# tingliu/glia

Measured on AMD Instinct MI355X. Metric: region_merges_per_sec, higher is better.
Workload: dtype u32 labels / f32 image / f64 statistics and features

## Files before the change

### glia_amd/csrc/api.cpp

```cpp
#include <algorithm>
#include <atomic>
#include <cmath>
#include <cstdlib>
#include <cstring>
#include <limits>
#include <mutex>
#include <unordered_map>

#include "rmap_order.hpp"
#include "api_types.hpp"

namespace glia {

static thread_local std::string g_err;
void set_error(const std::string& msg) { g_err = msg; }

static const char* const kOptionKeys[] = {"GLIA_HMT_PB_WINDOW", "GLIA_HMT_PB_BATCH", "GLIA_HMT_WINCAP", "GLIA_HMT_REBASE", "GLIA_HMT_HORIZON",
                                          "GLIA_HMT_FORCE_TREE", "GLIA_HMT_HELPERS", "GLIA_HMT_TRACE", "GLIA_HMT_LIBM", "GLIA_HMT_BC_NOCOMMON",
                                          "GLIA_HMT_BC_GENERIC", "GLIA_HMT_DEBUG", "GLIA_HMT_MAXITERS", "GLIA_HMT_MINCAP", "GLIA_HMT_MEDIAN_BATCH", "GLIA_HMT_BCFEAT", "GLIA_HMT_CC",
                                          "GLIA_HMT_TRAIN_TREES"};
static std::mutex g_opt_mu;
static std::unordered_map<std::string, std::string> g_opt;
static bool g_opt_init = false;
static void opt_init_locked() {
  if (g_opt_init) return;
  for (const char* k : kOptionKeys) if (const char* e = getenv(k)) g_opt[k] = e;
  g_opt_init = true;
}
static bool opt_known(const char* key) { for (const char* k : kOptionKeys) if (!strcmp(k, key)) return true; return false; }
bool option(const char* key, std::string* value) {
  std::lock_guard<std::mutex> lock(g_opt_mu);
  opt_init_locked();
  auto it = g_opt.find(key);
  if (it == g_opt.end()) return false;
  if (value) *value = it->second;
  return true;
}
int set_option(const char* key, const char* value) {
  if (!key || !opt_known(key)) { set_error(std::string("set_option: unknown option ") + (key ? key : "(null)")); return GLIA_HMT_ERR_ARG; }
  std::lock_guard<std::mutex> lock(g_opt_mu);
  opt_init_locked();
  if (value) g_opt[key] = value; else g_opt.erase(key);
  return GLIA_HMT_OK;
}

float ceil_f32(double d) {
  if (std::isinf(d) || std::isnan(d)) return (float)d;
  float f = (float)d;
  if ((double)f < d) f = std::nextafterf(f, std::numeric_limits<float>::infinity());
  return f;
}
static float floor_f32(double d) {
  if (std::isinf(d) || std::isnan(d)) return (float)d;
// ... 333 lines not shown
```

### glia_amd/csrc/greedy.hip

```cpp
#include <atomic>
#include <cstring>
#include <vector>
#include <limits>
#include <rocprim/device/device_scan.hpp>
#include <rocprim/device/device_radix_sort.hpp>
#include <rocprim/device/device_segmented_radix_sort.hpp>

#include "greedy_batch.hpp"

namespace glia {

__global__ void pq_build_level_kernel(PqTree t, int l) {
  const int lane = threadIdx.x & 63;
  uint32_t j = (blockIdx.x * blockDim.x + threadIdx.x) >> 6;
  if (j < t.lv[l].size) (void)pq_recompute_node(t, l, j, lane, true);
}

int pq_setup(DeviceBuffers& buf, PqTree& t, hipStream_t stream) {
  t.nlevels = 0;
  uint32_t n = t.nleaves;
  while (true) {
    n = (n + kFan - 1) / kFan;
    if (t.nlevels >= kMaxLevels) { set_error("greedy: edge table too large"); return GLIA_HMT_ERR_ARG; }
    PqLevel& L = t.lv[t.nlevels++];
// ... 14 lines not shown
  for (int l = 0; l < t.nlevels; ++l) {
    unsigned long long threads = (unsigned long long)t.lv[l].size * 64ull;
    hipLaunchKernelGGL(pq_build_level_kernel, dim3((unsigned)((threads + 255) / 256)), dim3(256), 0, stream, t, l);
  }
  GLIA_HIP_TRY(hipGetLastError());
  return GLIA_HMT_OK;
}

namespace {

__global__ void win_range_kernel(const double* sal, uint32_t E0, unsigned long long* mm) {
  unsigned long long lo = ~0ull, hi = 0ull;
  for (uint32_t i = blockIdx.x * blockDim.x + threadIdx.x; i < E0; i += gridDim.x * blockDim.x) {
    const unsigned long long b = f64_ord(sal[i]);
    lo = b < lo ? b : lo; hi = b > hi ? b : hi;
  }
  atomicMin(&mm[0], lo); atomicMax(&mm[1], hi);
}
__global__ void win_params_kernel(const unsigned long long* mm, uint32_t B, double* range) {
  const double smin = f64_unord(mm[0]), smax = f64_unord(mm[1]);
  range[0] = smin;
  range[1] = smax > smin ? (double)B / (smax - smin) : 0.0;
}
__global__ void win_collect_kernel(const EdgeRec* er, uint32_t n_edges, const uint8_t* rdead, unsigned long long* kseq, uint32_t* vals, uint32_t* counter) {
  const uint32_t e = blockIdx.x * blockDim.x + threadIdx.x;
  if (e >= n_edges) return;
  const unsigned long long q = er[e].seq;
  if (q == 0) return;
  const uint2 uv = *reinterpret_cast<const uint2*>(&er[e].u);
  if (rdead[uv.x] | rdead[uv.y]) return;
  const uint32_t i = atomicAdd(counter, 1u);
  kseq[i] = q; vals[i] = e;
}
__global__ void win_collect_lists_kernel(WinState st, uint32_t n_regions, unsigned long long* kseq, uint32_t* vals, uint32_t cap, uint32_t* counter) {
  const uint32_t r = (blockIdx.x * blockDim.x + threadIdx.x) >> 6, lane = threadIdx.x & 63u;
  if (r >= n_regions || st.rdead[r]) return;
  const uint32_t off = st.adj_off[r], len = st.adj_len[r];
  const double smin = st.wrange[0], scale = st.wrange[1];
  uint32_t rebuilt = 0;
  for (uint32_t base = 0; base < len; base += 64u) {
    const uint32_t i = base + lane;
    unsigned long long q = 0;
    uint32_t e = kNone;
    if (i < len) {
      const FatEntry fe = st.fpool[off + i];
      if (fe.eid != kNone && fe.rs < r && !st.rdead[fe.rs]) {
        e = fe.eid;
        if ((unsigned long long)e >= st.ne_base && win_cell(-fe.mean, smin, scale, st.wB) < st.wch) {
          const EdgeRec rec = rebuild_edge_record(fe, i, r, off, len, st.ecat[e], st.R0);
          st.er[e] = rec;
          q = rec.seq; ++rebuilt;
        } else q = st.er[e].seq;
      }
    }
    const unsigned long long m = __ballot(q != 0);
    if (m == 0) continue;
    const int first = (int)__builtin_ctzll(m);
    uint32_t b0 = 0;
    if ((int)lane == first) b0 = atomicAdd(&counter[0], (uint32_t)__popcll(m));
    b0 = (uint32_t)__shfl((int)b0, first);
    const uint32_t o = b0 + (uint32_t)__popcll(m & ((1ull << lane) - 1ull));
    if (q != 0 && o < cap) { kseq[o] = q; vals[o] = e; }
  }
  if (rebuilt) atomicAdd(&counter[1], rebuilt);
}
__global__ void win_salkey_kernel(const EdgeRec* er, const uint32_t* vals, uint32_t n, unsigned long long* ksal) {
  const uint32_t i = blockIdx.x * blockDim.x + threadIdx.x;
  if (i < n) ksal[i] = f64_ord(er[vals[i]].sal);
}
__global__ void win_baseline_fill_kernel(WinState st, uint32_t n, uint32_t* isort_w, unsigned long long* isort_seq) {
  const uint32_t i = blockIdx.x * blockDim.x + threadIdx.x;
  if (i >= n) return;
  const EdgeRec r = st.er[isort_w[i]];
  isort_seq[i] = r.seq;
  atomicAdd(&st.wcnt[win_cell(r.sal, st.wrange[0], st.wrange[1], st.wB)], 1u);
}
__global__ void win_segments_kernel(WinState st, const uint32_t* isort, uint32_t n, uint32_t* ige) {
  const uint32_t c = blockIdx.x * blockDim.x + threadIdx.x;
  if (c > st.wB) return;
  uint32_t lo = 0, hi = n;
  while (lo < hi) {
    const uint32_t mid = (lo + hi) >> 1;
    if (win_cell(st.er[isort[mid]].sal, st.wrange[0], st.wrange[1], st.wB) >= c) lo = mid + 1; else hi = mid;
  }
  ige[c] = c == 0 ? n : lo;
}
__global__ void adj_fill_fat(GreedyState g, WinState st, uint32_t E0, uint32_t* cursor) {
  const uint32_t e = blockIdx.x * blockDim.x + threadIdx.x;
  if (e >= E0) return;
  const uint32_t u = g.e_u[e], v = g.e_v[e];
  const uint32_t pu = atomicAdd(&cursor[u], 1u), pv = atomicAdd(&cursor[v], 1u);
  const uint32_t ou = g.adj_off[u], ov = g.adj_off[v], lu = g.adj_len[u], lv = g.adj_len[v];
  FatEntry a; a.eid = e; a.rs = v; a.n = (uint32_t)g.e_n[e]; a.pos = pv; a.off = ov; a.len = lv; a.mean = g.e_mean[e];
  FatEntry b = a; b.rs = u; b.pos = pu; b.off = ou; b.len = lu;
  st.fpool[ou + pu] = a; g.e_posu[e] = pu;
  st.fpool[ov + pv] = b; g.e_posv[e] = pv;
  EdgeRec r; r.u = u; r.v = v; r.posu = pu; r.posv = pv; r.mean = g.e_mean[e]; r.n = g.e_n[e]; r.next = kNone;
  r.hu = make_uint2(ou, lu); r.hv = make_uint2(ov, lv); r.sal = g.pq.leaf_sal[e]; r.seq = g.pq.leaf_seq[e];
  st.er[e] = r;
}
__global__ void fat_to_thin(const FatEntry* f, uint2* out, unsigned long long n) {
  const unsigned long long i = (unsigned long long)blockIdx.x * blockDim.x + threadIdx.x;
  if (i < n) { const FatEntry fe = f[i]; out[i] = make_uint2(fe.eid, fe.eid == kNone ? 0u : fe.rs); }
}
__global__ void edge_unpack(GreedyState g, const EdgeRec* er, const uint8_t* rdead, uint32_t n) {
  const uint32_t e = blockIdx.x * blockDim.x + threadIdx.x;
  if (e >= n) return;
  const EdgeRec r = er[e];
  g.e_u[e] = r.u; g.e_v[e] = r.v; g.e_posu[e] = r.posu; g.e_posv[e] = r.posv; g.e_mean[e] = r.mean; g.e_n[e] = r.n;
  g.pq.leaf_sal[e] = r.sal; g.pq.leaf_seq[e] = (rdead[r.u] | rdead[r.v]) ? 0ull : r.seq;
}

__global__ void edge_unpack_live(GreedyState g, const EdgeRec* er, const uint32_t* vals, uint32_t n) {
  const uint32_t i = blockIdx.x * blockDim.x + threadIdx.x;
  if (i >= n) return;
  const uint32_t e = vals[i];
  const EdgeRec r = er[e];
  g.e_u[e] = r.u; g.e_v[e] = r.v; g.e_posu[e] = r.posu; g.e_posv[e] = r.posv; g.e_mean[e] = r.mean; g.e_n[e] = r.n;
// ... 79 lines not shown
__global__ void median_from_runs(const unsigned long long* pv_off, const float* pv, unsigned long long nV, const uint32_t* pa, const uint32_t* pb, long long P,
                                 const uint32_t* flag, const uint32_t* eidx, const unsigned long long* e_off, float* out) {
  const unsigned long long v = (unsigned long long)blockIdx.x * blockDim.x + threadIdx.x;
  if (v >= nV) return;
  long long lo = 0, hi = P;
  while (lo < hi) { const long long mid = (lo + hi) >> 1; if (pv_off[mid + 1] <= v) lo = mid + 1; else hi = mid; }
  const long long i = lo;
  const uint32_t a = pa[i], b = pb[i];
  const long long owner = a < b ? i : find_pair(pa, pb, P, b, a);
  if (owner < 0 || !flag[owner]) return;
  const unsigned long long first = owner == i ? 0ull : pv_off[owner + 1] - pv_off[owner];
  out[e_off[eidx[owner]] + first + (v - pv_off[i])] = pv[v];
}

__global__ void median_init(GreedyState st, uint32_t E0) {
  const uint32_t e = blockIdx.x * blockDim.x + threadIdx.x;
  if (e >= E0) return;
  const uint32_t n = (uint32_t)st.e_n[e];
  const double med = (double)st.vals[st.e_off[e] + n / 2u];
  st.e_mean[e] = med;
  st.pq.leaf_sal[e] = st.size_weight ? -med * (double)min(st.rsz[st.e_u[e]], st.rsz[st.e_v[e]]) : -med;
  atomicAdd(&st.rbv[st.e_u[e]], (unsigned long long)n);
  atomicAdd(&st.rbv[st.e_v[e]], (unsigned long long)n);
}

__global__ void fill_leaves_dead(PqTree t, uint32_t from) {
  uint32_t i = from + blockIdx.x * blockDim.x + threadIdx.x;
  if (i < t.nleaves) { t.leaf_seq[i] = 0; t.leaf_sal[i] = -__builtin_inf(); }
}

}

struct WinBaseline {
  unsigned long long *kseq = nullptr, *kseq2 = nullptr, *ksal = nullptr, *ksal2 = nullptr, *iseq = nullptr;
  uint32_t *vals = nullptr, *vals2 = nullptr, *isort = nullptr, *ige = nullptr, *counter = nullptr;
  void* tmp = nullptr; size_t tmp_bytes = 0;
  uint32_t E0 = 0;
  double h_range[2] = {0.0, 0.0};
  long long prev_top_cell = -1;
  unsigned long long prev_ne = 0;
  double horizon_factor = 0.0;
  bool from_lists = false;
  unsigned long long rebuilt_last = 0;

  int init(DeviceBuffers& buf, WinState& ws, const double* leaf_sal, uint32_t n_initial, uint32_t B, uint32_t R, hipStream_t stream) {
    int rc;
    E0 = n_initial;
    unsigned long long* mm; double* range;
    if ((rc = buf.get(&ws.rdead, 2 * (size_t)R, true, stream))) return rc;
    if ((rc = buf.get(&ws.whead, B, false, stream))) return rc;
    if ((rc = buf.get(&ws.wcnt, B, true, stream))) return rc;
    if ((rc = buf.get(&isort, E0, false, stream))) return rc;
    if ((rc = buf.get(&iseq, E0, false, stream))) return rc;
    if ((rc = buf.get(&ige, (size_t)B + 1, false, stream))) return rc;
    if ((rc = buf.get(&mm, 2, false, stream))) return rc;
    if ((rc = buf.get(&range, 2, false, stream))) return rc;
    if ((rc = buf.get(&kseq, E0, false, stream))) return rc;
    if ((rc = buf.get(&kseq2, E0, false, stream))) return rc;
    if ((rc = buf.get(&ksal, E0, false, stream))) return rc;
    if ((rc = buf.get(&ksal2, E0, false, stream))) return rc;
    if ((rc = buf.get(&vals, E0, false, stream))) return rc;
    if ((rc = buf.get(&vals2, E0, false, stream))) return rc;
    if ((rc = buf.get(&counter, 2, true, stream))) return rc;
    GLIA_HIP_TRY(rocprim::radix_sort_pairs_desc(nullptr, tmp_bytes, kseq, kseq2, vals, vals2, (size_t)E0, 0, 64, stream));
    if ((rc = buf.get((char**)&tmp, tmp_bytes ? tmp_bytes : 16, false, stream))) return rc;
    ws.wrange = range; ws.isort = isort; ws.isort_seq = iseq; ws.ige = ige;
    const unsigned long long mm0[2] = {~0ull, 0ull};
    GLIA_HIP_TRY(hipMemcpyAsync(mm, mm0, sizeof(mm0), hipMemcpyHostToDevice, stream));
    hipLaunchKernelGGL(win_range_kernel, dim3(256), dim3(256), 0, stream, leaf_sal, E0, mm);
    hipLaunchKernelGGL(win_params_kernel, dim3(1), dim3(1), 0, stream, mm, B, range);
    GLIA_HIP_TRY(hipGetLastError());
    GLIA_HIP_TRY(hipMemcpyAsync(h_range, range, sizeof(h_range), hipMemcpyDeviceToHost, stream));
    GLIA_HIP_TRY(hipStreamSynchronize(stream));
    return GLIA_HMT_OK;
  }
  int collect(const WinState& ws, uint32_t n_edges, uint32_t n_regions, hipStream_t stream, uint32_t* n_out) {
    GLIA_HIP_TRY(hipMemsetAsync(counter, 0, 2 * sizeof(uint32_t), stream));
    if (from_lists) hipLaunchKernelGGL(win_collect_lists_kernel, dim3((unsigned)(((unsigned long long)n_regions * 64ull + 255ull) / 256ull)), dim3(256), 0, stream, ws, n_regions, kseq, vals, E0, counter);
    else hipLaunchKernelGGL(win_collect_kernel, dim3((n_edges + 255) / 256), dim3(256), 0, stream, ws.er, n_edges, ws.rdead, kseq, vals, counter);
    GLIA_HIP_TRY(hipGetLastError());
    uint32_t h[2] = {0, 0};
    GLIA_HIP_TRY(hipMemcpyAsync(h, counter, sizeof(h), hipMemcpyDeviceToHost, stream));
    GLIA_HIP_TRY(hipStreamSynchronize(stream));
    if (h[0] > E0) { set_error("greedy: more live edges than initial edges (internal error)"); return GLIA_HMT_ERR_INTERNAL; }
    *n_out = h[0]; rebuilt_last = h[1];
    return GLIA_HMT_OK;
  }
  int rebaseline(WinState& ws, uint32_t n_edges, unsigned long long* ctrl, hipStream_t stream) {
    uint32_t n = 0;
    if (int rc = collect(ws, n_edges, ws.R0 + (uint32_t)ctrl[CTRL_MERGES], stream, &n)) return rc;
    if (n) {
      size_t bytes = tmp_bytes;
      GLIA_HIP_TRY(rocprim::radix_sort_pairs_desc(tmp, bytes, kseq, kseq2, vals, vals2, (size_t)n, 0, 64, stream));
      hipLaunchKernelGGL(win_salkey_kernel, dim3((n + 255) / 256), dim3(256), 0, stream, ws.er, vals2, n, ksal);
      bytes = tmp_bytes;
      GLIA_HIP_TRY(rocprim::radix_sort_pairs_desc(tmp, bytes, ksal, ksal2, vals2, isort, (size_t)n, 0, 64, stream));
    }
    GLIA_HIP_TRY(hipMemsetAsync(ws.whead, 0xFF, sizeof(uint32_t) * ws.wB, stream));
    GLIA_HIP_TRY(hipMemsetAsync(ws.wcnt, 0, sizeof(uint32_t) * ws.wB, stream));
    if (n) hipLaunchKernelGGL(win_baseline_fill_kernel, dim3((n + 255) / 256), dim3(256), 0, stream, ws, n, isort, iseq);
    hipLaunchKernelGGL(win_segments_kernel, dim3((ws.wB + 1 + 255) / 256), dim3(256), 0, stream, ws, isort, n, ige);
    GLIA_HIP_TRY(hipGetLastError());
    ws.nsort = n;
    std::string renv;
    ws.rebase_after = option("GLIA_HMT_REBASE", &renv) ? strtoull(renv.c_str(), nullptr, 10) : std::max<unsigned long long>(800000ull, (unsigned long long)n / 2ull);
    ws.wch = 0;
    if (horizon_factor > 0.0 && n > 4096) {
      unsigned long long topkey = 0;
      GLIA_HIP_TRY(hipMemcpyAsync(&topkey, ksal2, sizeof(topkey), hipMemcpyDeviceToHost, stream));
      GLIA_HIP_TRY(hipStreamSynchronize(stream));
      const long long top_cell = (long long)win_cell(f64_unord(topkey), h_range[0], h_range[1], ws.wB);
      if (prev_top_cell >= 0 && n_edges > prev_ne) {
        const double d = (double)std::max<long long>(0, prev_top_cell - top_cell);
        const double delta = std::max(horizon_factor * d * (double)ws.rebase_after / (double)(n_edges - prev_ne), (double)ws.wB / 512.0);
        ws.wch = (double)top_cell > delta ? (uint32_t)((double)top_cell - delta) : 0u;
      }
      prev_top_cell = top_cell; prev_ne = n_edges;
    }
    ws.ne_base = n_edges;
    const double inf = std::numeric_limits<double>::infinity();
    ctrl[CTRL_CTHR] = (unsigned long long)(long long)(ws.wB - 1);
    memcpy(&ctrl[CTRL_TSAL], &inf, 8); ctrl[CTRL_TSEQ] = ~0ull; ctrl[CTRL_IPTR] = 0;
    return GLIA_HMT_OK;
  }
};

static int run_pb_loop(const RagArrays& rag, hipStream_t stream, const PbRequest& req, MergeResult* out) {
  const long long P = rag.P;
  const uint32_t R = (uint32_t)rag.R;
  if (R == 0 || P == 0) return GLIA_HMT_OK;
  const VolumeRef* median_of = req.median_of;
  CallEvents<3> ev;
  int rc;
  if ((rc = ev.create())) return rc;
  GLIA_HIP_TRY(hipEventRecord(ev.ev[0], stream));
  DeviceBuffers buf;
  uint32_t* flag; uint32_t* eidx; long long* partner;
  if ((rc = buf.get(&flag, P + 1, true, stream))) return rc;
  if ((rc = buf.get(&eidx, P + 1, false, stream))) return rc;
  if ((rc = buf.get(&partner, P, false, stream))) return rc;
  hipLaunchKernelGGL(edge_flags, dim3((unsigned)((P + 255) / 256)), dim3(256), 0, stream, rag.d_pa, rag.d_pb, P, flag, partner);
  if ((rc = rocprim_run(buf, stream, [&](void* t, size_t& b) {
        return rocprim::exclusive_scan(t, b, flag, eidx, 0u, (size_t)(P + 1), rocprim::plus<uint32_t>(), stream); }))) return rc;
  uint32_t E0 = 0;
  GLIA_HIP_TRY(hipMemcpyAsync(&E0, eidx + P, sizeof(uint32_t), hipMemcpyDeviceToHost, stream));
  GLIA_HIP_TRY(hipStreamSynchronize(stream));
  if (E0 == 0) return GLIA_HMT_OK;

  GreedyState st;
  memset(&st, 0, sizeof(st));
  st.R0 = R;
  const bool mincap = initial_capacities(E0, 18, 36, &st.Ecap, &st.pool_cap);
  if ((rc = buf.get(&st.adj_off, 2 * (size_t)R, true, stream))) return rc;
  if ((rc = buf.get(&st.adj_len, 2 * (size_t)R + 1, true, stream))) return rc;
  std::string o_window, o_batch, o_txt;
// ... 218 lines not shown
```

### glia_amd/csrc/greedy_batch.hpp

```cpp
#pragma once
#include "greedy_window.hpp"

namespace glia {
namespace {

constexpr uint32_t kBatchKill = 32;
constexpr int kMemP = 3;
constexpr uint32_t kMemMax = 192;
struct BatchShared {
  alignas(16) Key part1[kNW];
  alignas(16) Key part2[kNW];
  uint32_t nkill, kovf; alignas(16) uint32_t kill[kBatchKill];
  uint32_t byrank[kNW];
  uint32_t bitmap[kNW][64];
  uint32_t m_newcount[kNW], m_total[kNW], m_ok[kNW];
  double m_maxsal[kNW];
  uint32_t bad;
};

template <int CTRL, int ROW_MASK = 0xf>
__device__ __forceinline__ void top2_ord_step(unsigned long long& a1, unsigned long long& a2) {
  const unsigned long long b1 = dpp64<CTRL, ROW_MASK, ROW_MASK != 0xf>(a1), b2 = dpp64<CTRL, ROW_MASK, ROW_MASK != 0xf>(a2);
  const bool g = b1 > a1;
  const unsigned long long hi = g ? b1 : a1, lo = g ? a1 : b1, m2 = b2 > a2 ? b2 : a2;
// ... 435 lines not shown
        const uint32_t offRs = fe[p].off, posRs = fe[p].pos, lenRs = fe[p].len;
        if (both[p]) st.fpool[offRs + p_pos[p]].eid = kNone;
        const unsigned long long seq = update_seq(kk, rs, r0, h0);
        const double sal = -first[p];
        const uint32_t cell = win_cell(sal, tau.smin, tau.scale, st.wB);
#ifdef GLIA_HMT_PROFILE
        if (cell < st.wch) ++bep_below; else ++bep_above;
#endif
        store_new_edge<true>(st, newE, rs, r2, posRs, idx[p], first[p], second[p], sal, seq, offRs, lenRs, r2off, newcount, cell);
        win_queue_edge<true>(st, w, tau, newE, sal, seq, rs, r2, make_uint2(offRs, lenRs), make_uint2(r2off, newcount), cell, pend_e, pend_old);
        win_retire_edge<true, false, kBatchKill>(st, tau, fe[p].eid, -fe[p].mean, &b.nkill, b.kill, &b.kovf);
        if (both[p]) win_retire_edge<true, false, kBatchKill>(st, tau, p_eid[p], -p_mean[p], &b.nkill, b.kill, &b.kovf);
      }
    }
    lds_barrier();
    BPH(3);
#ifdef GLIA_HMT_PROFILE
    brounds += 1; bmembers += M; bvalid += V;
#endif
    k += V; ne += ne_off; pool_used += pool_off;
    batch_scan(st, w, b, tid, kScanNarrow);
    if (w.spill_ord) { if (pend_e != kNone) { st.er[pend_e].next = pend_old; pend_e = kNone; } win_evict(st, w, tid); batch_scan(st, w, b, tid, kScanOther); }
    BPH(4);
  }
#ifdef GLIA_HMT_PROFILE
  if (bep_above) atomicAdd(&g_edgeprof[0][0], (unsigned long long)bep_above);
  if (bep_below) atomicAdd(&g_edgeprof[0][1], (unsigned long long)bep_below);
  full_barrier();
  if (tid == 0) printf("[batch profile] created edges at or above / below the horizon (cumulative): narrow commit %llu / %llu  wide on the LDS table %llu / %llu  wide on the global marks %llu / %llu\n",
                       atomicAdd(&g_edgeprof[0][0], 0ull), atomicAdd(&g_edgeprof[0][1], 0ull), atomicAdd(&g_edgeprof[1][0], 0ull), atomicAdd(&g_edgeprof[1][1], 0ull),
                       atomicAdd(&g_edgeprof[2][0], 0ull), atomicAdd(&g_edgeprof[2][1], 0ull));
  if (tid == 0) printf("[batch profile] merges %llu: select %llu  compute %llu  validate %llu  commit %llu  scan %llu  loop-top %llu  reload %llu (cycles); rounds %llu candidates %llu committed %llu (cut by saliency %llu, by adjacency %llu) wide %llu\n",
                       k, bph[0], bph[1], bph[2], bph[3], bph[4], bph[5], bph[6], brounds, bmembers, bvalid, bcut_sal, bcut_dep, bwide);
  if (tid == 0) printf("[batch profile] scan phases (cumulative cycles, wave 0): loads %llu  compare %llu  top2 %llu  top2 with a tied best %llu  barrier %llu  calls %llu  tied second %llu  tied best %llu\n",
                       g_scanprof[0], g_scanprof[1], g_scanprof[2], g_scanprof[3], g_scanprof[4], g_scanprof[7], g_scanprof[5], g_scanprof[6]);
  if (tid == 0) printf("[batch profile] scan fill (cumulative; n <= 512, <= 1024, more): after reload/evict %llu %llu %llu  after narrow round %llu %llu %llu  after wide %llu %llu %llu\n",
                       g_scanfill[0][0], g_scanfill[0][1], g_scanfill[0][2], g_scanfill[1][0], g_scanfill[1][1], g_scanfill[1][2], g_scanfill[2][0], g_scanfill[2][1], g_scanfill[2][2]);
  if (tid == 0) printf("[batch profile] loop top (this launch): narrow rounds %llu cycles %llu  wide pops %llu cycles %llu\n", bsel_n[0], bsel[0], bsel_n[1], bsel[1]);
  if (tid == 0) printf("[batch profile] wide phases (cumulative cycles): entry-barrier %llu  lists+table %llu  compact %llu  main loop (wave 0) %llu  loop barrier %llu  tail %llu\n",
                       g_wideprof[0], g_wideprof[1], g_wideprof[2], g_wideprof[3], g_wideprof[4], g_wideprof[5]);
  if (tid == 0) printf("[batch profile] wide by entries (<=512, <=1408, <=8192, more): n %llu %llu %llu %llu  cycles %llu %llu %llu %llu  entries %llu %llu %llu %llu  new edges %llu %llu %llu %llu\n",
                       bw_n[0], bw_n[1], bw_n[2], bw_n[3], bw_cyc[0], bw_cyc[1], bw_cyc[2], bw_cyc[3], bw_ent[0], bw_ent[1], bw_ent[2], bw_ent[3], bw_new[0], bw_new[1], bw_new[2], bw_new[3]);
#endif
  if (pend_e != kNone) st.er[pend_e].next = pend_old;
  full_barrier();
  win_leave(st, w, tid, k, ne, pool_used, status);
}

}
}
```

### glia_amd/csrc/greedy_window.hpp

```cpp
#pragma once
#include "greedy_tree.hpp"
#include "edge_record.hpp"

namespace glia {
namespace {

static_assert(kRecNone == kNone, "edge_record.hpp");
struct WinState {
  EdgeRec* er; FatEntry* fpool;
  uint32_t* whead;
  uint32_t* wcnt;
  const uint32_t* isort; const unsigned long long* isort_seq;
  const uint32_t* ige;
  const double* wrange;
  uint32_t* order; double* sal_out; unsigned long long* ctrl;
  unsigned long long* rsz; double* rsum; uint32_t *mark0, *mark1, *adj_off, *adj_len;
  unsigned long long pool_cap, max_iters, cond_t0, cond_t1;
  double cond_rpb;
  uint32_t R0, Ecap, wB, nsort;
  unsigned long long ne_base, rebase_after;
  uint32_t wcap, wbudget;
  int cond_n;
  uint32_t wch;
  uint8_t* rdead;
// ... 140 lines not shown
    const uint32_t c = win_cell(w.sal[i], smin, scale, st.wB);
    win_push_global(st, w.e[i], c);
    mc = mc > c + 1u ? mc : c + 1u;
  }
  if (mc) atomicMax(&w.maxcell, mc);
  full_barrier();
  if (tid == 0) {
    if (w.maxcell && (int)w.maxcell - 1 >= w.cthr) { w.cthr = (int)w.maxcell - 1; w.tsal = __builtin_inf(); w.tseq = ~0ull; }
    w.n = 0;
  }
  full_barrier();
}

__device__ __forceinline__ void win_evict(const WinState& st, WinShared& w, int tid) {
  const double smin = st.wrange[0], scale = st.wrange[1];
  const double lim = f64_unord(w.spill_ord);
  const uint32_t n = w.n < st.wcap ? w.n : st.wcap;
  full_barrier();
  for (uint32_t i = tid; i < n; i += kGreedyThreads) {
    if (w.seq[i] == 0 || w.sal[i] > lim) continue;
    win_push_global(st, w.e[i], win_cell(w.sal[i], smin, scale, st.wB));
    w.seq[i] = 0;
  }
  full_barrier();
  if (tid == 0) { w.n = n; w.cthr = (int)win_cell(lim, smin, scale, st.wB); w.tsal = lim; w.tseq = ~0ull; w.spill_ord = 0; }
  full_barrier();
}

__device__ __forceinline__ void win_take_initial(const WinState& st, WinShared& w, uint32_t a, uint32_t b, int tid) {
  for (uint32_t i = a + (uint32_t)tid; i < b; i += kGreedyThreads) { const uint32_t e = st.isort[i]; const EdgeRec r = st.er[e]; win_take(st, w, e, r); }
}

constexpr uint32_t kSelMax = 384;
__device__ __forceinline__ int win_reload(const WinState& st, WinShared& w, int tid, double* sel_sal, unsigned long long* sel_seq) {
  full_barrier();
  if (tid == 0) { w.n = 0; w.need_tree = 0; }
  full_barrier();
  uint32_t c_hi = (uint32_t)(w.cthr + 1) < st.wB ? (uint32_t)(w.cthr + 1) : st.wB, loaded = 0, iptr = w.iptr;
  int result = 1;
  const uint32_t c_floor = st.wch < st.wB ? st.wch : 0u;
  while (c_hi > c_floor) {
    const bool valid = (uint32_t)tid < c_hi - c_floor;
    const uint32_t c = valid ? c_hi - 1u - (uint32_t)tid : 0u;
    const uint32_t cn = valid ? ld_relaxed(&st.wcnt[c]) : 0u;
    uint32_t total;
    const uint32_t incl = block_scan_incl(cn, w.wsum, tid, &total);
    const bool ok = valid && incl <= st.wbudget - loaded;
    const uint32_t m = (uint32_t)__syncthreads_count(ok ? 1 : 0);
    const uint32_t nvalid = c_hi - c_floor < (uint32_t)kGreedyThreads ? c_hi - c_floor : (uint32_t)kGreedyThreads;
    if (m != 0) {
      const uint32_t c_lo = c_hi - m;
      if ((uint32_t)tid == m - 1u) w.bcast = incl;
      const uint32_t i_to = st.ige[c_lo];
      win_take_initial(st, w, iptr, i_to, tid);
      iptr = i_to > iptr ? i_to : iptr;
      if ((uint32_t)tid < m) {
        uint32_t e = ld_relaxed(&st.whead[c]);
        if (e != kNone) {
          st_agent(&st.whead[c], kNone);
          if (cn != 0) while (e != kNone) { const EdgeRec r = st.er[e]; win_take(st, w, e, r); e = r.next; }
        }
        if (cn != 0) st_agent(&st.wcnt[c], 0u);
      }
      full_barrier();
      loaded += w.bcast;
      c_hi = c_lo;
      if (loaded) result = 0;
    }
    if (m < nvalid) {
      const uint32_t room = st.wbudget - loaded;
      const uint32_t cs = c_hi - 1u;
      if (room >= (kWinMinPartial < st.wbudget / 8u ? kWinMinPartial : st.wbudget / 8u) || loaded == 0) {
        const uint32_t K = (room / 2u < kSelMax ? room / 2u : kSelMax) > 1u ? (room / 2u < kSelMax ? room / 2u : kSelMax) : 2u, RA = room > K ? room - K : 1u;
        const uint32_t seg_end = st.ige[cs];
        const uint32_t before = w.n;
        if (tid == 0) {
          uint32_t hn = 0, nlive = 0;
          for (uint32_t e = ld_relaxed(&st.whead[cs]); e != kNone;) {
            const EdgeRec r = st.er[e];
            if (r.seq != 0) {
              ++nlive;
              if (hn < K) {
                uint32_t i = hn++;
                while (i > 0) {
                  const uint32_t p = (i - 1u) >> 1;
                  if (!(sel_sal[p] > r.sal || (sel_sal[p] == r.sal && sel_seq[p] > r.seq))) break;
                  sel_sal[i] = sel_sal[p]; sel_seq[i] = sel_seq[p]; i = p;
                }
                sel_sal[i] = r.sal; sel_seq[i] = r.seq;
              } else if (r.sal > sel_sal[0] || (r.sal == sel_sal[0] && r.seq > sel_seq[0])) {
                uint32_t i = 0;
                while (true) {
                  uint32_t c = 2u * i + 1u;
                  if (c >= hn) break;
                  if (c + 1u < hn && (sel_sal[c + 1u] < sel_sal[c] || (sel_sal[c + 1u] == sel_sal[c] && sel_seq[c + 1u] < sel_seq[c]))) ++c;
                  if (!(sel_sal[c] < r.sal || (sel_sal[c] == r.sal && sel_seq[c] < r.seq))) break;
                  sel_sal[i] = sel_sal[c]; sel_seq[i] = sel_seq[c]; i = c;
                }
                sel_sal[i] = r.sal; sel_seq[i] = r.seq;
              }
            }
// ... 8 lines not shown
          const uint32_t et = st.isort[iA]; const double as = st.er[et].sal; const unsigned long long aq = st.isort_seq[iA];
          if (as > tsal || (as == tsal && aq > tseq)) { tsal = as; tseq = aq; }
        }
        if (tid == 0) w.bcast = 0;
        full_barrier();
        uint32_t mine = 0;
        for (uint32_t i = iptr + (uint32_t)tid; i < iA; i += kGreedyThreads) {
          const uint32_t e = st.isort[i]; const EdgeRec r = st.er[e];
          const unsigned long long q = st.isort_seq[i];
          if (r.sal > tsal || (r.sal == tsal && q > tseq)) { ++mine; win_take(st, w, e, r); }
        }
        if (mine) atomicAdd(&w.bcast, mine);
        full_barrier();
        iptr += w.bcast;
        if (tid == 0) {
          uint32_t keep_head = kNone, keep_tail = kNone;
          for (uint32_t e = ld_relaxed(&st.whead[cs]); e != kNone;) {
            const EdgeRec r = st.er[e];
            if (r.seq != 0) {
              if (r.sal > tsal || (r.sal == tsal && r.seq > tseq)) win_take(st, w, e, r);
              else { if (keep_head == kNone) keep_head = e; else st.er[keep_tail].next = e; keep_tail = e; }
            }
            e = r.next;
          }
          if (keep_tail != kNone) st.er[keep_tail].next = kNone;
          st_agent(&st.whead[cs], keep_head);
        }
        full_barrier();
        const uint32_t moved = w.n - before;
        if (moved == 0u && w.bcast == 0u) {
          full_barrier();
          if (tid == 0) st_agent(&st.wcnt[cs], 0u);
          c_hi = cs;
          continue;
        }
        if (tid == 0) { if (moved) atomicSub(&st.wcnt[cs], moved); w.cthr = (int)cs; w.tsal = tsal; w.tseq = tseq; w.iptr = iptr; }
        if (moved || w.bcast) result = 0;
        full_barrier();
        return result;
      }
      break;
    }
    if (loaded >= (kWinMinLoad < st.wbudget / 4u ? kWinMinLoad : st.wbudget / 4u)) break;
  }
  full_barrier();
  if (tid == 0 && result != 2) { w.cthr = (int)c_hi - 1; w.tsal = __builtin_inf(); w.tseq = ~0ull; w.iptr = iptr; }
  full_barrier();
  if (result == 1 && c_floor != 0u) result = 3;
  return result;
}

struct WinTau { int cthr; double tsal; unsigned long long tseq; double smin, scale; };

__device__ __forceinline__ void win_stage_lists(const WinState& st, WinWork& s, int tid, uint32_t e, uint32_t off0, uint32_t len0, uint32_t off1, uint32_t len1, bool small) {
  const uint32_t total = len0 + len1;
  for (uint32_t i = tid; i < total; i += kGreedyThreads) {
    const bool side1 = i >= len0;
    const FatEntry fe = st.fpool[side1 ? off1 + (i - len0) : off0 + i];
    if (fe.eid == e || fe.eid == kNone) continue;
    if (small) {
      s.stage[i] = fe;
      uint32_t h = (fe.rs * 2654435761u) >> 21;
      while (true) {
        const uint32_t old = atomicCAS(&s.mk[h], 0u, fe.rs + 1u);
        if (old == 0u) { s.items[atomicAdd(&s.nitems, 1u)] = h; break; }
        if (old == fe.rs + 1u) break;
        h = (h + 1u) & (kMarkSlots - 1u);
      }
      (side1 ? s.mv1 : s.mv0)[h] = i + 1u;
    } else (side1 ? st.mark1 : st.mark0)[fe.rs] = i + 1u;
  }
// ... 313 lines not shown
```

Before: 328,100.

## Sort window baseline by index permutation and narrow seq radix bits

The window rebaseline now sorts an index permutation instead of edge ids. The saliency key is produced during collection (or by the salkey kernel on the non-list path), and the later fill and segment kernels read sorted keys directly instead of gathering EdgeRec records. The seq sort uses only as many radix bits as the region count requires. Short adjacency lists are walked with 16-lane groups chosen by a density heuristic, and the initial threshold cell is set to the top occupied cell. This also adds an optional audit kernel and reload profiling counters, at the cost of more buffers and added complexity.

```diff
diff --git a/glia_amd/csrc/api.cpp b/glia_amd/csrc/api.cpp
--- a/glia_amd/csrc/api.cpp
+++ b/glia_amd/csrc/api.cpp
@@ -18,7 +18,7 @@
 static const char* const kOptionKeys[] = {"GLIA_HMT_PB_WINDOW", "GLIA_HMT_PB_BATCH", "GLIA_HMT_WINCAP", "GLIA_HMT_REBASE", "GLIA_HMT_HORIZON",
                                           "GLIA_HMT_FORCE_TREE", "GLIA_HMT_HELPERS", "GLIA_HMT_TRACE", "GLIA_HMT_LIBM", "GLIA_HMT_BC_NOCOMMON",
                                           "GLIA_HMT_BC_GENERIC", "GLIA_HMT_DEBUG", "GLIA_HMT_MAXITERS", "GLIA_HMT_MINCAP", "GLIA_HMT_MEDIAN_BATCH", "GLIA_HMT_BCFEAT", "GLIA_HMT_CC",
-                                          "GLIA_HMT_TRAIN_TREES"};
+                                          "GLIA_HMT_TRAIN_TREES", "GLIA_HMT_BASELINE_AUDIT", "GLIA_HMT_COLLECT_LANES"};
 static std::mutex g_opt_mu;
 static std::unordered_map<std::string, std::string> g_opt;
 static bool g_opt_init = false;
diff --git a/glia_amd/csrc/greedy.hip b/glia_amd/csrc/greedy.hip
--- a/glia_amd/csrc/greedy.hip
+++ b/glia_amd/csrc/greedy.hip
@@ -70,20 +70,24 @@
   const uint32_t i = atomicAdd(counter, 1u);
   kseq[i] = q; vals[i] = e;
 }
-__global__ void win_collect_lists_kernel(WinState st, uint32_t n_regions, unsigned long long* kseq, uint32_t* vals, uint32_t cap, uint32_t* counter) {
-  const uint32_t r = (blockIdx.x * blockDim.x + threadIdx.x) >> 6, lane = threadIdx.x & 63u;
-  if (r >= n_regions || st.rdead[r]) return;
+struct CollectOut { unsigned long long *kseq, *ksal; uint32_t *vals, *idx, *counter; uint32_t cap; };
+template <uint32_t W>
+__device__ __forceinline__ uint32_t win_collect_walk(const WinState& st, const CollectOut& out, uint32_t r) {
+  static_assert(W == 16u || W == 64u, "lanes per list");
+  const uint32_t lane = threadIdx.x & 63u, gl = lane & (W - 1u), gshift = lane & ~(W - 1u);
+  const unsigned long long gmask = W == 64u ? ~0ull : ((1ull << W) - 1ull);
   const uint32_t off = st.adj_off[r], len = st.adj_len[r];
   const double smin = st.wrange[0], scale = st.wrange[1];
   uint32_t rebuilt = 0;
-  for (uint32_t base = 0; base < len; base += 64u) {
-    const uint32_t i = base + lane;
-    unsigned long long q = 0;
+  for (uint32_t base = 0; base < len; base += W) {
+    const uint32_t i = base + gl;
+    unsigned long long q = 0, sk = 0;
     uint32_t e = kNone;
     if (i < len) {
       const FatEntry fe = st.fpool[off + i];
       if (fe.eid != kNone && fe.rs < r && !st.rdead[fe.rs]) {
         e = fe.eid;
+        sk = f64_ord(-fe.mean);
         if ((unsigned long long)e >= st.ne_base && win_cell(-fe.mean, smin, scale, st.wB) < st.wch) {
           const EdgeRec rec = rebuild_edge_record(fe, i, r, off, len, st.ecat[e], st.R0);
           st.er[e] = rec;
@@ -91,37 +95,83 @@
         } else q = st.er[e].seq;
       }
     }
-    const unsigned long long m = __ballot(q != 0);
+    const unsigned long long m = (__ballot(e != kNone) >> gshift) & gmask;
     if (m == 0) continue;
     const int first = (int)__builtin_ctzll(m);
     uint32_t b0 = 0;
-    if ((int)lane == first) b0 = atomicAdd(&counter[0], (uint32_t)__popcll(m));
-    b0 = (uint32_t)__shfl((int)b0, first);
-    const uint32_t o = b0 + (uint32_t)__popcll(m & ((1ull << lane) - 1ull));
-    if (q != 0 && o < cap) { kseq[o] = q; vals[o] = e; }
-  }
-  if (rebuilt) atomicAdd(&counter[1], rebuilt);
-}
-__global__ void win_salkey_kernel(const EdgeRec* er, const uint32_t* vals, uint32_t n, unsigned long long* ksal) {
+    if ((int)gl == first) b0 = atomicAdd(&out.counter[0], (uint32_t)__popcll(m));
+    b0 = (uint32_t)__shfl((int)b0, (int)gshift + first);
+    const uint32_t o = b0 + (uint32_t)__popcll(m & ((1ull << gl) - 1ull));
+    if (e != kNone && o < out.cap) { out.kseq[o] = q; out.ksal[o] = sk; out.vals[o] = e; out.idx[o] = o; }
+  }
+  return rebuilt;
+}
+constexpr uint32_t kCollectShort = 32;
+template <uint32_t G>
+__global__ void win_collect_lists_kernel(WinState st, uint32_t n_regions, CollectOut out) {
+  const uint32_t t = blockIdx.x * blockDim.x + threadIdx.x;
+  uint32_t rebuilt = 0;
+  if constexpr (G == 64u) {
+    const uint32_t r = t >> 6;
+    if (r >= n_regions || st.rdead[r]) return;
+    rebuilt = win_collect_walk<64u>(st, out, r);
+  } else {
+    const uint32_t r = t / G;
+    if (r < n_regions && !st.rdead[r] && st.adj_len[r] <= kCollectShort) rebuilt = win_collect_walk<G>(st, out, r);
+    for (uint32_t j = 0; j < 64u / G; ++j) {
+      const uint32_t rj = (t >> 6) * (64u / G) + j;
+      if (rj < n_regions && !st.rdead[rj] && st.adj_len[rj] > kCollectShort) rebuilt += win_collect_walk<64u>(st, out, rj);
+    }
+  }
+  if (rebuilt) atomicAdd(&out.counter[1], rebuilt);
+}
+__global__ void win_salkey_kernel(const EdgeRec* er, const uint32_t* vals, uint32_t n, unsigned long long* ksal, uint32_t* idx) {
   const uint32_t i = blockIdx.x * blockDim.x + threadIdx.x;
-  if (i < n) ksal[i] = f64_ord(er[vals[i]].sal);
-}
-__global__ void win_baseline_fill_kernel(WinState st, uint32_t n, uint32_t* isort_w, unsigned long long* isort_seq) {
+  if (i < n) { ksal[i] = f64_ord(er[vals[i]].sal); idx[i] = i; }
+}
+__global__ void win_gather_key_kernel(const unsigned long long* ksal, const uint32_t* idx, uint32_t n, unsigned long long* out) {
+  const uint32_t i = blockIdx.x * blockDim.x + threadIdx.x;
+  if (i < n) out[i] = ksal[idx[i]];
+}
+__global__ void win_baseline_fill_kernel(WinState st, uint32_t n, const unsigned long long* ksal_sorted, const uint32_t* idx, const unsigned long long* kseq, const uint32_t* vals,
+                                         uint32_t* isort_w, unsigned long long* isort_seq) {
   const uint32_t i = blockIdx.x * blockDim.x + threadIdx.x;
   if (i >= n) return;
-  const EdgeRec r = st.er[isort_w[i]];
-  isort_seq[i] = r.seq;
-  atomicAdd(&st.wcnt[win_cell(r.sal, st.wrange[0], st.wrange[1], st.wB)], 1u);
-}
-__global__ void win_segments_kernel(WinState st, const uint32_t* isort, uint32_t n, uint32_t* ige) {
+  const uint32_t j = idx[i];
+  isort_w[i] = vals[j]; isort_seq[i] = kseq[j];
+  atomicAdd(&st.wcnt[win_cell(f64_unord(ksal_sorted[i]), st.wrange[0], st.wrange[1], st.wB)], 1u);
+}
+__global__ void win_segments_kernel(WinState st, const unsigned long long* ksal_sorted, uint32_t n, uint32_t* ige) {
   const uint32_t c = blockIdx.x * blockDim.x + threadIdx.x;
   if (c > st.wB) return;
   uint32_t lo = 0, hi = n;
   while (lo < hi) {
     const uint32_t mid = (lo + hi) >> 1;
-    if (win_cell(st.er[isort[mid]].sal, st.wrange[0], st.wrange[1], st.wB) >= c) lo = mid + 1; else hi = mid;
+    if (win_cell(f64_unord(ksal_sorted[mid]), st.wrange[0], st.wrange[1], st.wB) >= c) lo = mid + 1; else hi = mid;
   }
   ige[c] = c == 0 ? n : lo;
+}
+__global__ void win_baseline_audit_kernel(WinState st, uint32_t n, const unsigned long long* kseq, const unsigned long long* ksal, const uint32_t* vals,
+                                          const unsigned long long* ksal_sorted, const uint32_t* isort, const unsigned long long* iseq, const uint32_t* ige,
+                                          long long cthr, uint32_t* bad) {
+  const uint32_t i = blockIdx.x * blockDim.x + threadIdx.x;
+  uint32_t wrong = 0;
+  if (i < n) {
+    const EdgeRec a = st.er[vals[i]];
+    wrong += a.seq != kseq[i] || f64_ord(a.sal) != ksal[i] || kseq[i] == 0;
+    const EdgeRec b = st.er[isort[i]];
+    const unsigned long long ks = ksal_sorted[i], q = iseq[i];
+    wrong += b.seq != q || f64_ord(b.sal) != ks;
+    if (i > 0) wrong += ksal_sorted[i - 1] < ks || (ksal_sorted[i - 1] == ks && iseq[i - 1] <= q);
+    const uint32_t c = win_cell(f64_unord(ks), st.wrange[0], st.wrange[1], st.wB);
+    wrong += (long long)c > cthr;
+    wrong += !(ige[c + 1] <= i && i < ige[c]);
+  }
+  if (i <= st.wB) {
+    wrong += i == 0 ? ige[0] != n : ige[i] > ige[i - 1];
+    if (i < st.wB) wrong += ige[i] < ige[i + 1] || st.wcnt[i] != ige[i] - ige[i + 1];
+  }
+  if (wrong) atomicAdd(bad, wrong);
 }
 __global__ void adj_fill_fat(GreedyState g, WinState st, uint32_t E0, uint32_t* cursor) {
   const uint32_t e = blockIdx.x * blockDim.x + threadIdx.x;
@@ -267,20 +317,24 @@
 }
 
 struct WinBaseline {
-  unsigned long long *kseq = nullptr, *kseq2 = nullptr, *ksal = nullptr, *ksal2 = nullptr, *iseq = nullptr;
-  uint32_t *vals = nullptr, *vals2 = nullptr, *isort = nullptr, *ige = nullptr, *counter = nullptr;
+  unsigned long long *kseq = nullptr, *kseq2 = nullptr, *ksal = nullptr, *ksalg = nullptr, *ksal2 = nullptr, *iseq = nullptr;
+  uint32_t *vals = nullptr, *idx = nullptr, *idx1 = nullptr, *idx2 = nullptr, *isort = nullptr, *ige = nullptr, *counter = nullptr;
   void* tmp = nullptr; size_t tmp_bytes = 0;
   uint32_t E0 = 0;
   double h_range[2] = {0.0, 0.0};
   long long prev_top_cell = -1;
   unsigned long long prev_ne = 0;
+  uint32_t n_last = 0;
   double horizon_factor = 0.0;
   bool from_lists = false;
   unsigned long long rebuilt_last = 0;
+  int seq_bits = 64;
+  uint32_t lanes_forced = 0;
+  bool audit = false;
 
   int init(DeviceBuffers& buf, WinState& ws, const double* leaf_sal, uint32_t n_initial, uint32_t B, uint32_t R, hipStream_t stream) {
     int rc;
-    E0 = n_initial;
+    E0 = n_initial; n_last = n_initial;
     unsigned long long* mm; double* range;
     if ((rc = buf.get(&ws.rdead, 2 * (size_t)R, true, stream))) return rc;
     if ((rc = buf.get(&ws.whead, B, false, stream))) return rc;
@@ -293,11 +347,20 @@
     if ((rc = buf.get(&kseq, E0, false, stream))) return rc;
     if ((rc = buf.get(&kseq2, E0, false, stream))) return rc;
     if ((rc = buf.get(&ksal, E0, false, stream))) return rc;
+    if ((rc = buf.get(&ksalg, E0, false, stream))) return rc;
     if ((rc = buf.get(&ksal2, E0, false, stream))) return rc;
     if ((rc = buf.get(&vals, E0, false, stream))) return rc;
-    if ((rc = buf.get(&vals2, E0, false, stream))) return rc;
-    if ((rc = buf.get(&counter, 2, true, stream))) return rc;
-    GLIA_HIP_TRY(rocprim::radix_sort_pairs_desc(nullptr, tmp_bytes, kseq, kseq2, vals, vals2, (size_t)E0, 0, 64, stream));
+    if ((rc = buf.get(&idx, E0, false, stream))) return rc;
+    if ((rc = buf.get(&idx1, E0, false, stream))) return rc;
+    if ((rc = buf.get(&idx2, E0, false, stream))) return rc;
+    if ((rc = buf.get(&counter, 3, true, stream))) return rc;
+    GLIA_HIP_TRY(rocprim::radix_sort_pairs_desc(nullptr, tmp_bytes, kseq, kseq2, idx, idx1, (size_t)E0, 0, 64, stream));
+    seq_bits = 33;
+    while (seq_bits < 63 && ((unsigned long long)R >> (seq_bits - 32)) != 0) ++seq_bits;
+    seq_bits += 1;
+    std::string o_txt;
+    if (option("GLIA_HMT_COLLECT_LANES", &o_txt)) lanes_forced = (uint32_t)strtoul(o_txt.c_str(), nullptr, 10);
+    audit = option("GLIA_HMT_BASELINE_AUDIT", &o_txt) && o_txt[0] != '0';
     if ((rc = buf.get((char**)&tmp, tmp_bytes ? tmp_bytes : 16, false, stream))) return rc;
     ws.wrange = range; ws.isort = isort; ws.isort_seq = iseq; ws.ige = ige;
     const unsigned long long mm0[2] = {~0ull, 0ull};
@@ -310,15 +373,22 @@
     return GLIA_HMT_OK;
   }
   int collect(const WinState& ws, uint32_t n_edges, uint32_t n_regions, hipStream_t stream, uint32_t* n_out) {
-    GLIA_HIP_TRY(hipMemsetAsync(counter, 0, 2 * sizeof(uint32_t), stream));
-    if (from_lists) hipLaunchKernelGGL(win_collect_lists_kernel, dim3((unsigned)(((unsigned long long)n_regions * 64ull + 255ull) / 256ull)), dim3(256), 0, stream, ws, n_regions, kseq, vals, E0, counter);
-    else hipLaunchKernelGGL(win_collect_kernel, dim3((n_edges + 255) / 256), dim3(256), 0, stream, ws.er, n_edges, ws.rdead, kseq, vals, counter);
+    GLIA_HIP_TRY(hipMemsetAsync(counter, 0, 3 * sizeof(uint32_t), stream));
+    if (from_lists) {
+      const unsigned long long live_regions = 2ull * ws.R0 > n_regions ? 2ull * ws.R0 - n_regions : 1ull;
+      const uint32_t G = lanes_forced == 16u || lanes_forced == 64u ? lanes_forced : 2ull * n_last <= 24ull * live_regions ? 16u : 64u;
+      const dim3 grid((unsigned)(((unsigned long long)n_regions * G + 255ull) / 256ull));
+      const CollectOut out = {kseq, ksal, vals, idx, counter, E0};
+      if (G == 16u) hipLaunchKernelGGL(win_collect_lists_kernel<16u>, grid, dim3(256), 0, stream, ws, n_regions, out);
+      else hipLaunchKernelGGL(win_collect_lists_kernel<64u>, grid, dim3(256), 0, stream, ws, n_regions, out);
+    } else hipLaunchKernelGGL(win_collect_kernel, dim3((n_edges + 255) / 256), dim3(256), 0, stream, ws.er, n_edges, ws.rdead, kseq, vals, counter);
     GLIA_HIP_TRY(hipGetLastError());
     uint32_t h[2] = {0, 0};
     GLIA_HIP_TRY(hipMemcpyAsync(h, counter, sizeof(h), hipMemcpyDeviceToHost, stream));
     GLIA_HIP_TRY(hipStreamSynchronize(stream));
     if (h[0] > E0) { set_error("greedy: more live edges than initial edges (internal error)"); return GLIA_HMT_ERR_INTERNAL; }
-    *n_out = h[0]; rebuilt_last = h[1];
+    *n_out = h[0]; rebuilt_last = h[1]; n_last = h[0];
+    if (!from_lists && h[0]) { hipLaunchKernelGGL(win_salkey_kernel, dim3((h[0] + 255) / 256), dim3(256), 0, stream, ws.er, vals, h[0], ksal, idx); GLIA_HIP_TRY(hipGetLastError()); }
     return GLIA_HMT_OK;
   }
   int rebaseline(WinState& ws, uint32_t n_edges, unsigned long long* ctrl, hipStream_t stream) {
@@ -326,25 +396,28 @@
     if (int rc = collect(ws, n_edges, ws.R0 + (uint32_t)ctrl[CTRL_MERGES], stream, &n)) return rc;
     if (n) {
       size_t bytes = tmp_bytes;
-      GLIA_HIP_TRY(rocprim::radix_sort_pairs_desc(tmp, bytes, kseq, kseq2, vals, vals2, (size_t)n, 0, 64, stream));
-      hipLaunchKernelGGL(win_salkey_kernel, dim3((n + 255) / 256), dim3(256), 0, stream, ws.er, vals2, n, ksal);
+      GLIA_HIP_TRY(rocprim::radix_sort_pairs_desc(tmp, bytes, kseq, kseq2, idx, idx1, (size_t)n, 0, (unsigned)seq_bits, stream));
+      hipLaunchKernelGGL(win_gather_key_kernel, dim3((n + 255) / 256), dim3(256), 0, stream, ksal, idx1, n, ksalg);
       bytes = tmp_bytes;
-      GLIA_HIP_TRY(rocprim::radix_sort_pairs_desc(tmp, bytes, ksal, ksal2, vals2, isort, (size_t)n, 0, 64, stream));
+      GLIA_HIP_TRY(rocprim::radix_sort_pairs_desc(tmp, bytes, ksalg, ksal2, idx1, idx2, (size_t)n, 0, 64, stream));
     }
     GLIA_HIP_TRY(hipMemsetAsync(ws.whead, 0xFF, sizeof(uint32_t) * ws.wB, stream));
     GLIA_HIP_TRY(hipMemsetAsync(ws.wcnt, 0, sizeof(uint32_t) * ws.wB, stream));
-    if (n) hipLaunchKernelGGL(win_baseline_fill_kernel, dim3((n + 255) / 256), dim3(256), 0, stream, ws, n, isort, iseq);
-    hipLaunchKernelGGL(win_segments_kernel, dim3((ws.wB + 1 + 255) / 256), dim3(256), 0, stream, ws, isort, n, ige);
+    if (n) hipLaunchKernelGGL(win_baseline_fill_kernel, dim3((n + 255) / 256), dim3(256), 0, stream, ws, n, ksal2, idx2, kseq, vals, isort, iseq);
+    hipLaunchKernelGGL(win_segments_kernel, dim3((ws.wB + 1 + 255) / 256), dim3(256), 0, stream, ws, ksal2, n, ige);
     GLIA_HIP_TRY(hipGetLastError());
     ws.nsort = n;
     std::string renv;
     ws.rebase_after = option("GLIA_HMT_REBASE", &renv) ? strtoull(renv.c_str(), nullptr, 10) : std::max<unsigned long long>(800000ull, (unsigned long long)n / 2ull);
     ws.wch = 0;
-    if (horizon_factor > 0.0 && n > 4096) {
+    long long top_cell = (long long)ws.wB - 1;
+    if (n) {
       unsigned long long topkey = 0;
       GLIA_HIP_TRY(hipMemcpyAsync(&topkey, ksal2, sizeof(topkey), hipMemcpyDeviceToHost, stream));
       GLIA_HIP_TRY(hipStreamSynchronize(stream));
-      const long long top_cell = (long long)win_cell(f64_unord(topkey), h_range[0], h_range[1], ws.wB);
+      top_cell = (long long)win_cell(f64_unord(topkey), h_range[0], h_range[1], ws.wB);
+    }
+    if (horizon_factor > 0.0 && n > 4096) {
       if (prev_top_cell >= 0 && n_edges > prev_ne) {
         const double d = (double)std::max<long long>(0, prev_top_cell - top_cell);
         const double delta = std::max(horizon_factor * d * (double)ws.rebase_after / (double)(n_edges - prev_ne), (double)ws.wB / 512.0);
@@ -354,8 +427,17 @@
     }
     ws.ne_base = n_edges;
     const double inf = std::numeric_limits<double>::infinity();
-    ctrl[CTRL_CTHR] = (unsigned long long)(long long)(ws.wB - 1);
+    ctrl[CTRL_CTHR] = (unsigned long long)top_cell;
     memcpy(&ctrl[CTRL_TSAL], &inf, 8); ctrl[CTRL_TSEQ] = ~0ull; ctrl[CTRL_IPTR] = 0;
+    if (audit) {
+      hipLaunchKernelGGL(win_baseline_audit_kernel, dim3((std::max(n, ws.wB + 1u) + 255u) / 256u), dim3(256), 0, stream, ws, n, kseq, ksal, vals, ksal2, isort, iseq, ige,
+                         top_cell, counter + 2);
+      GLIA_HIP_TRY(hipGetLastError());
+      uint32_t bad = 0;
+      GLIA_HIP_TRY(hipMemcpyAsync(&bad, counter + 2, sizeof(bad), hipMemcpyDeviceToHost, stream));
+      GLIA_HIP_TRY(hipStreamSynchronize(stream));
+      if (bad) { set_error("greedy: the baseline audit found " + std::to_string(bad) + " mismatches (internal error)"); return GLIA_HMT_ERR_INTERNAL; }
+    }
     return GLIA_HMT_OK;
   }
 };
diff --git a/glia_amd/csrc/greedy_batch.hpp b/glia_amd/csrc/greedy_batch.hpp
--- a/glia_amd/csrc/greedy_batch.hpp
+++ b/glia_amd/csrc/greedy_batch.hpp
@@ -491,6 +491,8 @@
                        atomicAdd(&g_edgeprof[2][0], 0ull), atomicAdd(&g_edgeprof[2][1], 0ull));
   if (tid == 0) printf("[batch profile] merges %llu: select %llu  compute %llu  validate %llu  commit %llu  scan %llu  loop-top %llu  reload %llu (cycles); rounds %llu candidates %llu committed %llu (cut by saliency %llu, by adjacency %llu) wide %llu\n",
                        k, bph[0], bph[1], bph[2], bph[3], bph[4], bph[5], bph[6], brounds, bmembers, bvalid, bcut_sal, bcut_dep, bwide);
+  if (tid == 0) printf("[batch profile] reload parts (cumulative cycles, thread 0): descent over blocks that load nothing %llu  whole-cell loads %llu  cell split %llu;  empty blocks %llu  reloads %llu\n",
+                       g_reloadprof[0], g_reloadprof[1], g_reloadprof[2], g_reloadprof[3], g_reloadprof[4]);
   if (tid == 0) printf("[batch profile] scan phases (cumulative cycles, wave 0): loads %llu  compare %llu  top2 %llu  top2 with a tied best %llu  barrier %llu  calls %llu  tied second %llu  tied best %llu\n",
                        g_scanprof[0], g_scanprof[1], g_scanprof[2], g_scanprof[3], g_scanprof[4], g_scanprof[7], g_scanprof[5], g_scanprof[6]);
   if (tid == 0) printf("[batch profile] scan fill (cumulative; n <= 512, <= 1024, more): after reload/evict %llu %llu %llu  after narrow round %llu %llu %llu  after wide %llu %llu %llu\n",
diff --git a/glia_amd/csrc/greedy_window.hpp b/glia_amd/csrc/greedy_window.hpp
--- a/glia_amd/csrc/greedy_window.hpp
+++ b/glia_amd/csrc/greedy_window.hpp
@@ -196,6 +196,12 @@
 }
 
 constexpr uint32_t kSelMax = 384;
+#ifdef GLIA_HMT_PROFILE
+__device__ unsigned long long g_reloadprof[5];
+#define RELOAD_T(i) do { if (tid == 0) { const unsigned long long tn_ = __builtin_readcyclecounter(); g_reloadprof[i] += tn_ - rl_; rl_ = tn_; } } while (0)
+#else
+#define RELOAD_T(i) do {} while (0)
+#endif
 __device__ __forceinline__ int win_reload(const WinState& st, WinShared& w, int tid, double* sel_sal, unsigned long long* sel_seq) {
   full_barrier();
   if (tid == 0) { w.n = 0; w.need_tree = 0; }
@@ -203,6 +209,10 @@
   uint32_t c_hi = (uint32_t)(w.cthr + 1) < st.wB ? (uint32_t)(w.cthr + 1) : st.wB, loaded = 0, iptr = w.iptr;
   int result = 1;
   const uint32_t c_floor = st.wch < st.wB ? st.wch : 0u;
+#ifdef GLIA_HMT_PROFILE
+  unsigned long long rl_ = __builtin_readcyclecounter();
+  if (tid == 0) g_reloadprof[4] += 1;
+#endif
   while (c_hi > c_floor) {
     const bool valid = (uint32_t)tid < c_hi - c_floor;
     const uint32_t c = valid ? c_hi - 1u - (uint32_t)tid : 0u;
@@ -230,7 +240,11 @@
       loaded += w.bcast;
       c_hi = c_lo;
       if (loaded) result = 0;
-    }
+#ifdef GLIA_HMT_PROFILE
+      if (w.bcast == 0u) { if (tid == 0) g_reloadprof[3] += 1; RELOAD_T(0); }
+      else RELOAD_T(1);
+#endif
+    } else RELOAD_T(0);
     if (m < nvalid) {
       const uint32_t room = st.wbudget - loaded;
       const uint32_t cs = c_hi - 1u;
@@ -305,11 +319,13 @@
           full_barrier();
           if (tid == 0) st_agent(&st.wcnt[cs], 0u);
           c_hi = cs;
+          RELOAD_T(2);
           continue;
         }
         if (tid == 0) { if (moved) atomicSub(&st.wcnt[cs], moved); w.cthr = (int)cs; w.tsal = tsal; w.tseq = tseq; w.iptr = iptr; }
         if (moved || w.bcast) result = 0;
         full_barrier();
+        RELOAD_T(2);
         return result;
       }
       break;
```

Result: faster. 335,600, median of 6 (+2.3%).
